# smdogroup/eigd

Measured on AMD Instinct MI355X. Metric: adjoint_mode_derivatives_per_sec, higher is better.
Workload: dtype f64

## Files before the change

### eigd_amd/csrc/sparse.hip

```cpp
#include <algorithm>
#include <cstdint>
#include <vector>

#include "common.h"

struct eigd_mat {
  eigd_ctx* ctx = nullptr;
  int n = 0;
  int ncols = 0;
  int64_t nnz = 0;
  int32_t* indptr = nullptr;
  int32_t* indices = nullptr;
  double* data = nullptr;
  int32_t* rowblocks = nullptr;
  int nblocks = 0;
  int ntiles = 0, umax = 0;
  int tnz_cap = 0;
  int32_t* tile_ptr = nullptr;
  int32_t* ucols = nullptr;
  uint16_t* lidx = nullptr;
};

namespace eigd {

constexpr int kTileRows = 32;
constexpr int kTileLds = 40 * 1024;
constexpr int kTileNnz = 1024;
constexpr int kNnzTile = 2048;
constexpr int kMaxRowsTile = 256;


__device__ __forceinline__ int xcd_remap(int b, int nblocks_padded) {
  const int per = nblocks_padded >> 3;
  return (b & 7) * per + (b >> 3);
}

__global__ __launch_bounds__(kThreads) void spmv_stream_kernel(const int32_t* __restrict__ rowblocks, int nblocks,
                                                              int nblocks_padded,
                                                              const int32_t* __restrict__ indptr,
                                                              const int32_t* __restrict__ indices,
                                                              const double* __restrict__ vals,
                                                              const double* __restrict__ x, double* __restrict__ y,
                                                              double alpha, double beta) {
  __shared__ double prod[kNnzTile];
  __shared__ double red[kThreads];
  const int b = xcd_remap(blockIdx.x, nblocks_padded);
  if (b >= nblocks) return;
  const int tid = threadIdx.x;
  const int r0 = rowblocks[b], r1 = rowblocks[b + 1];
  const int e0 = indptr[r0], e1 = indptr[r1];
  if (e1 - e0 <= kNnzTile - 2) {
    constexpr int IT = kNnzTile / (2 * kThreads);
    const int eb = e0 & ~1;
    typedef double dbl2 __attribute__((ext_vector_type(2)));
    typedef int int2v __attribute__((ext_vector_type(2)));
    dbl2 v[IT];
    int2v col[IT];
    double xa[IT], xb[IT];
#pragma unroll
    for (int it = 0; it < IT; ++it) {
      const int e = eb + 2 * (tid + it * kThreads);
      if (e < e1) {
        v[it] = __builtin_nontemporal_load(reinterpret_cast<const dbl2*>(vals + e));
        col[it] = __builtin_nontemporal_load(reinterpret_cast<const int2v*>(indices + e));
      } else {
        v[it] = dbl2{0.0, 0.0};
        col[it] = int2v{0, 0};
      }
    }
#pragma unroll
    for (int it = 0; it < IT; ++it) {
      const int e = eb + 2 * (tid + it * kThreads);
      xa[it] = (e >= e0 && e < e1) ? x[col[it][0]] : 0.0;
      xb[it] = (e + 1 < e1) ? x[col[it][1]] : 0.0;
    }
#pragma unroll
    for (int it = 0; it < IT; ++it) {
      const int e = eb + 2 * (tid + it * kThreads);
      if (e >= e0 && e < e1) prod[e - e0] = __dmul_rn(v[it][0], xa[it]);
      if (e + 1 < e1) prod[e + 1 - e0] = __dmul_rn(v[it][1], xb[it]);
    }
    __syncthreads();
    for (int r = r0 + tid; r < r1; r += kThreads) {
      const int a = indptr[r] - e0, z = indptr[r + 1] - e0;
      double s = 0.0;
      for (int q = a; q < z; ++q) s = __dadd_rn(s, prod[q]);
      y[r] = (beta == 0.0) ? alpha * s : alpha * s + beta * y[r];
    }
  } else {
    double s = 0.0;
    for (int e = e0 + tid; e < e1; e += kThreads) s += vals[e] * x[indices[e]];
    red[tid] = s;
    __syncthreads();
    for (int w = kThreads / 2; w > 0; w >>= 1) {
      if (tid < w) red[tid] += red[tid + w];
      __syncthreads();
    }
    if (tid == 0) y[r0] = (beta == 0.0) ? alpha * red[0] : alpha * red[0] + beta * y[r0];
  }
}

template <int KP>
__global__ __launch_bounds__(kThreads) void spmm_rows_kernel(int n, int k, const int32_t* __restrict__ indptr,
                                                            const int32_t* __restrict__ indices,
                                                            const double* __restrict__ vals,
                                                            const double* __restrict__ X, int ldx,
                                                            double* __restrict__ Y, int ldy, double alpha,
                                                            double beta) {
  constexpr int RP = kThreads / KP;
  const int c = threadIdx.x % KP;
  const int r = blockIdx.x * RP + threadIdx.x / KP;
  if (r >= n || c >= k) return;
  const int a = indptr[r], z = indptr[r + 1];
  double s = 0.0;
  int e = a;
  for (; e + 8 <= z; e += 8) {
    int col[8];
    double v[8], x[8];
#pragma unroll
    for (int q = 0; q < 8; ++q) {
      col[q] = indices[e + q];
      v[q] = vals[e + q];
    }
#pragma unroll
    for (int q = 0; q < 8; ++q) x[q] = X[static_cast<int64_t>(col[q]) * ldx + c];
#pragma unroll
    for (int q = 0; q < 8; ++q) s = __dadd_rn(s, __dmul_rn(v[q], x[q]));
  }
  for (; e < z; ++e) s = __dadd_rn(s, __dmul_rn(vals[e], X[static_cast<int64_t>(indices[e]) * ldx + c]));
  double* yp = Y + static_cast<int64_t>(r) * ldy + c;
  *yp = (beta == 0.0) ? alpha * s : alpha * s + beta * (*yp);
}

template <int KP, int LANES = 8>
struct SpmmTile {
  static constexpr int CPL = (KP >= LANES) ? KP / LANES : 1;
  static constexpr int LPR = KP / CPL;
  static constexpr int LD = (CPL >= 2) ? KP + 4 : KP + 1;
};

template <int KP, int LANES, bool DOTS = false>
__global__ __launch_bounds__(kThreads) void spmm_tiled_kernel(int n, int k, int ntiles, int tiles_per_xcd,
                                                             const int32_t* __restrict__ tile_ptr,
                                                             const int32_t* __restrict__ ucols,
                                                             const int32_t* __restrict__ indptr,
                                                             const uint16_t* __restrict__ lidx,
                                                             const double* __restrict__ vals,
                                                             const double* __restrict__ X, int ldx,
                                                             double* __restrict__ Y, int ldy, double alpha, double beta,
                                                             int umax, int tnz_cap,
                                                             const double* __restrict__ R = nullptr, int ldr = 0,
                                                             double* __restrict__ dots = nullptr) {
  extern __shared__ __align__(16) double Xs[];
  constexpr int RP = kThreads / KP;
  constexpr int CPL = SpmmTile<KP, LANES>::CPL, LPR = SpmmTile<KP, LANES>::LPR, LD = SpmmTile<KP, LANES>::LD;
  constexpr int RPP = kThreads / LPR;
  constexpr int NR = (kTileRows + RPP - 1) / RPP;
  double* const Vs = Xs + static_cast<size_t>(umax) * LD;
  uint16_t* const Ls = reinterpret_cast<uint16_t*>(Vs + tnz_cap);
  const int tile = (blockIdx.x & 7) * tiles_per_xcd + (blockIdx.x >> 3);
  if (tile >= ntiles) return;
  const int c = threadIdx.x % KP, rr = threadIdx.x / KP;
  const int pl = threadIdx.x % LPR, prow = threadIdx.x / LPR;
  const int u0 = tile_ptr[tile], nu = tile_ptr[tile + 1] - u0;
  const int rend = min(n, (tile + 1) * kTileRows);
  const int e0 = indptr[tile * kTileRows], tnz = indptr[rend] - e0;
  const bool staged = tnz <= tnz_cap;
  constexpr int NQ = kTileNnz / kThreads;
  int ra[NR], rz[NR];
#pragma unroll
  for (int i = 0; i < NR; ++i) {
    const int r = tile * kTileRows + prow + i * RPP;
    ra[i] = (r < rend) ? indptr[r] - e0 : 0;
    rz[i] = (r < rend) ? indptr[r + 1] - e0 : 0;
  }
  double sv[NQ];
  uint16_t sl[NQ];
#pragma unroll
  for (int q = 0; q < NQ; ++q) {
    const int e = threadIdx.x + q * kThreads;
    const bool ok = staged && e < tnz;
    sv[q] = ok ? vals[e0 + e] : 0.0;
    sl[q] = ok ? lidx[e0 + e] : uint16_t(0);
  }
  [[maybe_unused]] double xo[CPL], ro[CPL];
  if constexpr (DOTS) {
    const int r = tile * kTileRows + prow;
#pragma unroll
    for (int t = 0; t < CPL; ++t) {
      const bool ok = r < rend && CPL * pl + t < k;
      xo[t] = ok ? X[static_cast<int64_t>(r) * ldx + CPL * pl + t] : 0.0;
      ro[t] = ok ? R[static_cast<int64_t>(r) * ldr + CPL * pl + t] : 0.0;
    }
  }
  constexpr int SU = 16;
  for (int j0 = 0; j0 < nu; j0 += SU * RP) {
    int col[SU];
    double x[SU];
#pragma unroll
    for (int q = 0; q < SU; ++q) {
      const int j = j0 + q * RP + rr;
      col[q] = (j < nu) ? ucols[u0 + j] : -1;
    }
#pragma unroll
    for (int q = 0; q < SU; ++q) x[q] = (col[q] >= 0 && c < k) ? X[static_cast<int64_t>(col[q]) * ldx + c] : 0.0;
#pragma unroll
    for (int q = 0; q < SU; ++q) {
      const int j = j0 + q * RP + rr;
      if (j < nu) Xs[j * LD + c] = x[q];
    }
  }
  if (staged) {
#pragma unroll
    for (int q = 0; q < NQ; ++q) {
      const int e = threadIdx.x + q * kThreads;
      if (e < tnz) {
        Vs[e] = sv[q];
        Ls[e] = sl[q];
      }
    }
  }
  __syncthreads();
  const int cb = CPL * pl;
  if (!DOTS && cb >= k) return;
  [[maybe_unused]] double dzr[CPL], dzy[CPL];
  [[maybe_unused]] __shared__ double dred[DOTS ? (kThreads / 64) * 2 * KP : 1];
  if constexpr (DOTS) {
#pragma unroll
    for (int t = 0; t < CPL; ++t) dzr[t] = dzy[t] = 0.0;
  }
  auto finish_dots = [&]() {
    if constexpr (DOTS) {
      static_assert(KP >= LANES && NR == 1, "one pass over the tile's rows, eight lanes per row");
#pragma unroll
      for (int t = 0; t < CPL; ++t) {
#pragma unroll
        for (int off = LPR; off < 64; off <<= 1) {
          dzr[t] += __shfl_xor(dzr[t], off, 64);
          dzy[t] += __shfl_xor(dzy[t], off, 64);
        }
      }
      const int wave = threadIdx.x >> 6, lane = threadIdx.x & 63;
      if (lane < LPR) {
#pragma unroll
        for (int t = 0; t < CPL; ++t) {
          dred[(wave * 2 + 0) * KP + cb + t] = dzr[t];
          dred[(wave * 2 + 1) * KP + cb + t] = dzy[t];
        }
      }
      __syncthreads();
      if (threadIdx.x < 2 * k) {
        const int q = threadIdx.x / k, c2 = threadIdx.x % k;
        double v = 0.0;
#pragma unroll
        for (int w = 0; w < kThreads / 64; ++w) v += dred[(w * 2 + q) * KP + c2];
        dots[static_cast<int64_t>(tile) * 2 * k + threadIdx.x] = v;
      }
    }
  };
  auto store_row = [&](int r, const double (&s)[CPL]) {
    double* yp = Y + static_cast<int64_t>(r) * ldy + cb;
#pragma unroll
    for (int t = 0; t < CPL; ++t)
      if (cb + t < k) {
        const double yv = (beta == 0.0) ? alpha * s[t] : alpha * s[t] + beta * yp[t];
        yp[t] = yv;
        if constexpr (DOTS) {
          dzr[t] += xo[t] * ro[t];
          dzy[t] += xo[t] * yv;
        }
      }
  };
  const bool active = cb < k;
  if (active && staged) {
#pragma unroll
    for (int i = 0; i < NR; ++i) {
      const int r = tile * kTileRows + prow + i * RPP;
      if (r >= rend) break;
      const int a = ra[i], z = rz[i];
      double s[CPL];
#pragma unroll
      for (int t = 0; t < CPL; ++t) s[t] = 0.0;
      int e = a;
      for (; e + 8 <= z; e += 8) {
        int li[8];
        double v[8], x[8][CPL];
#pragma unroll
        for (int q = 0; q < 8; ++q) {
          li[q] = Ls[e + q];
          v[q] = Vs[e + q];
        }
#pragma unroll
        for (int q = 0; q < 8; ++q) {
          const double* xp = Xs + li[q] * LD + cb;
          if constexpr (CPL >= 2) {
            const double2* xp2 = reinterpret_cast<const double2*>(xp);
#pragma unroll
            for (int t = 0; t < CPL / 2; ++t) {
              const double2 w = xp2[t];
              x[q][2 * t] = w.x;
              x[q][2 * t + 1] = w.y;
            }
          } else {
            x[q][0] = xp[0];
          }
        }
#pragma unroll
        for (int q = 0; q < 8; ++q)
#pragma unroll
          for (int t = 0; t < CPL; ++t) s[t] = __dadd_rn(s[t], __dmul_rn(v[q], x[q][t]));
      }
      for (; e < z; ++e) {
        const double v = Vs[e];
        const double* xp = Xs + Ls[e] * LD + cb;
#pragma unroll
        for (int t = 0; t < CPL; ++t) s[t] = __dadd_rn(s[t], __dmul_rn(v, xp[t]));
      }
      store_row(r, s);
    }
  } else if (active) {
  for (int r = tile * kTileRows + prow; r < rend; r += RPP) {
    const int a = indptr[r], z = indptr[r + 1];
    double s[CPL];
#pragma unroll
    for (int t = 0; t < CPL; ++t) s[t] = 0.0;
    for (int e = a; e < z; ++e) {
      const double v = vals[e];
      const double* xp = Xs + lidx[e] * LD + cb;
#pragma unroll
      for (int t = 0; t < CPL; ++t) s[t] = __dadd_rn(s[t], __dmul_rn(v, xp[t]));
    }
    store_row(r, s);
  }
  }
  finish_dots();
}

__global__ __launch_bounds__(kThreads) void tile_dots_reduce_kernel(const double* __restrict__ dots, int ntiles, int nout,
                                                                   double* __restrict__ out) {
  __shared__ double red[kThreads];
  const int per = kThreads / nout;
  const int o = threadIdx.x % nout, sub = threadIdx.x / nout;
  double v = 0.0;
  if (sub < per)
    for (int t = blockIdx.x * per + sub; t < ntiles; t += gridDim.x * per) v += dots[static_cast<int64_t>(t) * nout + o];
  red[threadIdx.x] = v;
  __syncthreads();
  if (threadIdx.x < nout) {
    double t = 0.0;
    for (int q = 0; q < per; ++q) t += red[q * nout + threadIdx.x];
    out[static_cast<int64_t>(blockIdx.x) * nout + threadIdx.x] = t;
  }
}

}

using namespace eigd;

extern "C" {

int eigd_csr_upload(eigd_ctx* ctx, int n, int64_t nnz, const int32_t* hindptr, const int32_t* hindices,
                    const double* hdata, eigd_mat** out) {
  return eigd_csr_upload_rect(ctx, n, n, nnz, hindptr, hindices, hdata, out);
}

int eigd_csr_upload_rect(eigd_ctx* ctx, int n, int ncols, int64_t nnz, const int32_t* hindptr, const int32_t* hindices,
                         const double* hdata, eigd_mat** out) {
  EIGD_REQUIRE(ctx && hindptr && hindices && hdata && out, "null argument");
  EIGD_REQUIRE(n > 0 && ncols > 0 && nnz >= 0 && nnz < (int64_t(1) << 31), "bad matrix size %d x %d nnz=%lld", n, ncols,
               (long long)nnz);
  EIGD_REQUIRE(hindptr[0] == 0 && hindptr[n] == nnz, "indptr does not match nnz");
  for (int i = 0; i < n; ++i) EIGD_REQUIRE(hindptr[i + 1] >= hindptr[i], "indptr not monotone at row %d", i);
  for (int64_t e = 0; e < nnz; ++e)
    EIGD_REQUIRE(hindices[e] >= 0 && hindices[e] < ncols, "column index out of range at entry %lld", (long long)e);
  *out = nullptr;
  std::vector<int32_t> rb;
  rb.push_back(0);
  {
    int r = 0;
    while (r < n) {
      int start = r;
      int64_t cnt = 0;
      while (r < n && (r - start) < kMaxRowsTile) {
        int64_t len = hindptr[r + 1] - hindptr[r];
        if (cnt + len > kNnzTile - 2) break;
        cnt += len;
        ++r;
      }
      if (r == start) ++r;
      rb.push_back(r);
    }
  }
  const int ntiles = (n + kTileRows - 1) / kTileRows;
  std::vector<int32_t> tile_ptr(static_cast<size_t>(ntiles) + 1, 0), ucols;
  std::vector<uint16_t> lidx(static_cast<size_t>(nnz) + 8, 0);
  int umax = 0;
  int64_t tnz_max = 0;
  bool tiles_ok = true;
  {
    std::vector<int32_t> cols, stamp(static_cast<size_t>(ncols), -1), pos(static_cast<size_t>(ncols), 0);
    ucols.reserve(static_cast<size_t>(nnz) / 4 + 16);
    for (int t = 0; t < ntiles && tiles_ok; ++t) {
      const int r0 = t * kTileRows, r1 = std::min(n, r0 + kTileRows);
      cols.clear();
      for (int64_t e = hindptr[r0]; e < hindptr[r1]; ++e) {
        const int32_t cidx = hindices[e];
        if (stamp[cidx] != t) {
          stamp[cidx] = t;
          cols.push_back(cidx);
        }
      }
      std::sort(cols.begin(), cols.end());
      if (cols.size() > 65535) tiles_ok = false;
      umax = std::max<int>(umax, static_cast<int>(cols.size()));
      tnz_max = std::max<int64_t>(tnz_max, hindptr[r1] - hindptr[r0]);
      for (size_t q = 0; q < cols.size(); ++q) pos[cols[q]] = static_cast<int32_t>(q);
      for (int64_t e = hindptr[r0]; e < hindptr[r1]; ++e) lidx[e] = static_cast<uint16_t>(pos[hindices[e]]);
      ucols.insert(ucols.end(), cols.begin(), cols.end());
      tile_ptr[t + 1] = static_cast<int32_t>(ucols.size());
    }
  }
  EIGD_HIP(hipSetDevice(ctx->device));
  eigd_mat* A = new eigd_mat();
  A->ctx = ctx;
  A->n = n;
  A->ncols = ncols;
  A->nnz = nnz;
  A->nblocks = static_cast<int>(rb.size()) - 1;
  if (tiles_ok) {
    A->ntiles = ntiles;
    A->umax = umax;
    A->tnz_cap = static_cast<int>(std::min<int64_t>(kTileNnz, (tnz_max + 7) & ~int64_t(7)));
    hipError_t t1 = hipMalloc(reinterpret_cast<void**>(&A->tile_ptr), sizeof(int32_t) * tile_ptr.size());
    hipError_t t2 = hipMalloc(reinterpret_cast<void**>(&A->ucols), sizeof(int32_t) * std::max<size_t>(ucols.size(), 1));
    hipError_t t3 = hipMalloc(reinterpret_cast<void**>(&A->lidx), sizeof(uint16_t) * lidx.size());
    if (t1 != hipSuccess || t2 != hipSuccess || t3 != hipSuccess) {
      eigd_mat_free(A);
      set_error("hipMalloc failed for the SpMM tiles (n=%d nnz=%lld)", n, (long long)nnz);
      return EIGD_E_HIP;
    }
    EIGD_HIP(hipMemcpy(A->tile_ptr, tile_ptr.data(), sizeof(int32_t) * tile_ptr.size(), hipMemcpyHostToDevice));
    if (!ucols.empty()) EIGD_HIP(hipMemcpy(A->ucols, ucols.data(), sizeof(int32_t) * ucols.size(), hipMemcpyHostToDevice));
    EIGD_HIP(hipMemcpy(A->lidx, lidx.data(), sizeof(uint16_t) * lidx.size(), hipMemcpyHostToDevice));
  }
  hipError_t e1 = hipMalloc(reinterpret_cast<void**>(&A->indptr), sizeof(int32_t) * (n + 1));
  hipError_t e2 = hipMalloc(reinterpret_cast<void**>(&A->indices), sizeof(int32_t) * (nnz + 4));
  hipError_t e3 = hipMalloc(reinterpret_cast<void**>(&A->data), sizeof(double) * (nnz + 4));
  hipError_t e4 = hipMalloc(reinterpret_cast<void**>(&A->rowblocks), sizeof(int32_t) * rb.size());
  if (e1 != hipSuccess || e2 != hipSuccess || e3 != hipSuccess || e4 != hipSuccess) {
    eigd_mat_free(A);
    set_error("hipMalloc failed for CSR matrix (n=%d nnz=%lld)", n, (long long)nnz);
    return EIGD_E_HIP;
  }
  EIGD_HIP(hipMemcpy(A->indptr, hindptr, sizeof(int32_t) * (n + 1), hipMemcpyHostToDevice));
  if (nnz > 0) {
    EIGD_HIP(hipMemcpy(A->indices, hindices, sizeof(int32_t) * nnz, hipMemcpyHostToDevice));
    EIGD_HIP(hipMemcpy(A->data, hdata, sizeof(double) * nnz, hipMemcpyHostToDevice));
  }
  EIGD_HIP(hipMemcpy(A->rowblocks, rb.data(), sizeof(int32_t) * rb.size(), hipMemcpyHostToDevice));
  *out = A;
  return EIGD_OK;
}

int eigd_csr_update_values(eigd_mat* A, const double* hdata) {
  EIGD_REQUIRE(A && hdata, "null argument");
  EIGD_HIP(hipStreamSynchronize(A->ctx->stream));
  if (A->nnz > 0) EIGD_HIP(hipMemcpy(A->data, hdata, sizeof(double) * A->nnz, hipMemcpyHostToDevice));
  return EIGD_OK;
}

int eigd_csr_update_values_dev(eigd_mat* A, const double* dvals) {
  EIGD_REQUIRE(A && dvals, "null argument");
  if (A->nnz > 0)
    EIGD_HIP(hipMemcpyAsync(A->data, dvals, sizeof(double) * A->nnz, hipMemcpyDeviceToDevice, A->ctx->stream));
  return EIGD_OK;
}

int eigd_mat_free(eigd_mat* A) {
  if (!A) return EIGD_OK;
  if (A->ctx && A->ctx->stream) (void)hipStreamSynchronize(A->ctx->stream);
  if (A->indptr) (void)hipFree(A->indptr);
  if (A->indices) (void)hipFree(A->indices);
  if (A->data) (void)hipFree(A->data);
  if (A->rowblocks) (void)hipFree(A->rowblocks);
  if (A->tile_ptr) (void)hipFree(A->tile_ptr);
  if (A->ucols) (void)hipFree(A->ucols);
  if (A->lidx) (void)hipFree(A->lidx);
  delete A;
  return EIGD_OK;
}

int eigd_spmm(eigd_mat* A, const double* dX, int ldx, double* dY, int ldy, int k, double alpha, double beta) {
  EIGD_REQUIRE(A, "null argument");
  return eigd_spmm_on(A->ctx, A, dX, ldx, dY, ldy, k, alpha, beta);
}

int eigd_spmm_on(eigd_ctx* ctx, eigd_mat* A, const double* dX, int ldx, double* dY, int ldy, int k, double alpha,
                 double beta) {
  EIGD_REQUIRE(ctx && A && dX && dY, "null argument");
  EIGD_REQUIRE(ctx->device == A->ctx->device, "context and matrix live on different devices");
  EIGD_REQUIRE(k >= 1 && ldx >= k && ldy >= k, "bad block shape k=%d ldx=%d ldy=%d", k, ldx, ldy);
  EIGD_REQUIRE(dX != dY, "spmm cannot run in place");
  hipStream_t st = ctx->stream;
  if (k == 1 && ldx == 1 && ldy == 1) {
    const int nbp = (A->nblocks + 7) & ~7;
    hipLaunchKernelGGL(spmv_stream_kernel, dim3(nbp), dim3(kThreads), 0, st, A->rowblocks, A->nblocks, nbp, A->indptr,
                       A->indices, A->data, dX, dY, alpha, beta);
    EIGD_LAUNCH_CHECK();
    return EIGD_OK;
  }
  auto tile_fits = [&](int kpv) {
    const int cplv = (kpv >= 8) ? kpv / 8 : 1;
    return A->ntiles > 0 && sizeof(double) * static_cast<size_t>(A->umax) * (cplv >= 2 ? kpv + 4 : kpv + 1) <= static_cast<size_t>(kTileLds);
  };
  const int chunk = (k > 32 && !tile_fits(64) && tile_fits(32)) ? 32 : kMaxK;
  for (int c0 = 0; c0 < k; c0 += chunk) {
    const int kb = std::min(chunk, k - c0);
    const int kp = std::max(2, next_pow2(kb));
    const int rp = kThreads / kp;
    const dim3 grid((A->n + rp - 1) / rp);
    const int cpl = (kp >= 8) ? kp / 8 : 1;
    const size_t tile_lds = sizeof(double) * static_cast<size_t>(A->umax) * (cpl >= 2 ? kp + 4 : kp + 1);
    const size_t tile_lds_all = tile_lds + static_cast<size_t>(A->tnz_cap) * (sizeof(double) + sizeof(uint16_t));
    if (A->ntiles > 0 && tile_lds <= static_cast<size_t>(kTileLds)) {
      const int per_xcd = (A->ntiles + 7) / 8;
      const dim3 tgrid(per_xcd * 8);
#define EIGD_SPMM_TILED(KP)                                                                                            \
  case KP:                                                                                                             \
    hipLaunchKernelGGL((spmm_tiled_kernel<KP, 8>), tgrid, dim3(kThreads), tile_lds_all, st, A->n, kb, A->ntiles,       \
                       per_xcd, A->tile_ptr, A->ucols, A->indptr, A->lidx, A->data, dX + c0, ldx, dY + c0, ldy,        \
                       alpha, beta, A->umax, A->tnz_cap);                                                              \
    break;
      switch (kp) {
        EIGD_SPMM_TILED(2)
        EIGD_SPMM_TILED(4)
        EIGD_SPMM_TILED(8)
        EIGD_SPMM_TILED(16)
        EIGD_SPMM_TILED(32)
        EIGD_SPMM_TILED(64)
        default:
          set_error("internal: unexpected kp=%d", kp);
          return EIGD_E_INTERNAL;
      }
#undef EIGD_SPMM_TILED
      EIGD_LAUNCH_CHECK();
      continue;
    }
#define EIGD_SPMM_CASE(KP)                                                                                          \
  case KP:                                                                                                          \
    hipLaunchKernelGGL(spmm_rows_kernel<KP>, grid, dim3(kThreads), 0, st, A->n, kb, A->indptr, A->indices, A->data, \
                       dX + c0, ldx, dY + c0, ldy, alpha, beta);                                                    \
    break;
    switch (kp) {
      EIGD_SPMM_CASE(2)
      EIGD_SPMM_CASE(4)
      EIGD_SPMM_CASE(8)
      EIGD_SPMM_CASE(16)
      EIGD_SPMM_CASE(32)
      EIGD_SPMM_CASE(64)
      default:
        set_error("internal: unexpected kp=%d", kp);
        return EIGD_E_INTERNAL;
    }
#undef EIGD_SPMM_CASE
    EIGD_LAUNCH_CHECK();
  }
  return EIGD_OK;
}

int eigd_spmm_cg(eigd_ctx* ctx, eigd_mat* A, int k, const double* dZ, int ldz, double* dY, int ldy, const double* dR, int ldr,
                 const double* dNorm2, double* dState, int step, int first, double* dLog) {
  EIGD_REQUIRE(ctx && A && dZ && dY && dR && dState, "null argument");
  EIGD_REQUIRE(ctx->device == A->ctx->device, "context and matrix live on different devices");
  EIGD_REQUIRE(k >= 1 && k <= kMaxK && ldz >= k && ldy >= k && ldr >= k && A->n == A->ncols, "bad block shape k=%d", k);
  EIGD_REQUIRE(dZ != dY, "spmm cannot run in place");
  const int kp = std::max(2, next_pow2(k));
  const int cpl = (kp >= 8) ? kp / 8 : 1;
  const size_t tile_lds = sizeof(double) * static_cast<size_t>(A->umax) * (cpl >= 2 ? kp + 4 : kp + 1);
  const bool fused = kp >= 8 && kp <= 32 && A->ntiles > 0 && tile_lds <= static_cast<size_t>(kTileLds);
  if (!fused) {
    int rc = eigd_spmm_on(ctx, A, dZ, ldz, dY, ldy, k, 1.0, 0.0);
    if (rc) return rc;
    return eigd_cg_coefficients(ctx, A->n, k, dZ, ldz, dR, ldr, dY, ldy, dNorm2, dState, step, first, dLog);
  }
  const int groups = std::min(A->ntiles, 1024);
  int rc = ctx->ensure_scratch(sizeof(double) * (static_cast<size_t>(A->ntiles) + groups) * 2 * k);
  if (rc) return rc;
  double* gsum = ctx->scratch;
  double* dots = ctx->scratch + static_cast<size_t>(groups) * 2 * k;
  const size_t tile_lds_all = tile_lds + static_cast<size_t>(A->tnz_cap) * (sizeof(double) + sizeof(uint16_t));
  const int per_xcd = (A->ntiles + 7) / 8;
  const dim3 tgrid(per_xcd * 8);
  hipStream_t st = ctx->stream;
#define EIGD_SPMM_DOTS(KP)                                                                                             \
  case KP:                                                                                                             \
    hipLaunchKernelGGL((spmm_tiled_kernel<KP, 8, true>), tgrid, dim3(kThreads), tile_lds_all, st, A->n, k, A->ntiles,  \
                       per_xcd, A->tile_ptr, A->ucols, A->indptr, A->lidx, A->data, dZ, ldz, dY, ldy, 1.0, 0.0,        \
                       A->umax, A->tnz_cap, dR, ldr, dots);                                                            \
    break;
  switch (kp) {
    EIGD_SPMM_DOTS(8)
    EIGD_SPMM_DOTS(16)
    EIGD_SPMM_DOTS(32)
    default:
      set_error("internal: unexpected kp=%d", kp);
      return EIGD_E_INTERNAL;
  }
#undef EIGD_SPMM_DOTS
  EIGD_LAUNCH_CHECK();
  hipLaunchKernelGGL(tile_dots_reduce_kernel, dim3(groups), dim3(kThreads), 0, st, dots, A->ntiles, 2 * k, gsum);
  EIGD_LAUNCH_CHECK();
  return cg_coefficients_from_partials(ctx, gsum, groups, k, dNorm2, dState, step, first, dLog);
}

}
```

Measured before the change: 667.5.

## Pad per-tile column lists and hoist gather loads ahead of value staging

Replaces the tile_ptr indirection with a fixed-stride padded ucols array, so each tile's column list starts at tile*umax and the dependent tile_ptr load disappears. The first batch of column indices and X gathers is issued before the vals/lidx staging loads, and those loads are made unconditional through clamped indices so more memory requests are in flight at once. The gather batch size now adapts to rows per pass. In exchange, padded tiles gather up to umax columns even when the tile holds fewer, which adds wasted work on irregular matrices. A host check also disables tiling when padding would inflate memory too much.

```diff
diff --git a/eigd_amd/csrc/sparse.hip b/eigd_amd/csrc/sparse.hip
--- a/eigd_amd/csrc/sparse.hip
+++ b/eigd_amd/csrc/sparse.hip
@@ -16,7 +16,6 @@
   int nblocks = 0;
   int ntiles = 0, umax = 0;
   int tnz_cap = 0;
-  int32_t* tile_ptr = nullptr;
   int32_t* ucols = nullptr;
   uint16_t* lidx = nullptr;
 };
@@ -141,7 +140,6 @@
 
 template <int KP, int LANES, bool DOTS = false>
 __global__ __launch_bounds__(kThreads) void spmm_tiled_kernel(int n, int k, int ntiles, int tiles_per_xcd,
-                                                             const int32_t* __restrict__ tile_ptr,
                                                              const int32_t* __restrict__ ucols,
                                                              const int32_t* __restrict__ indptr,
                                                              const uint16_t* __restrict__ lidx,
@@ -162,53 +160,69 @@
   if (tile >= ntiles) return;
   const int c = threadIdx.x % KP, rr = threadIdx.x / KP;
   const int pl = threadIdx.x % LPR, prow = threadIdx.x / LPR;
-  const int u0 = tile_ptr[tile], nu = tile_ptr[tile + 1] - u0;
-  const int rend = min(n, (tile + 1) * kTileRows);
-  const int e0 = indptr[tile * kTileRows], tnz = indptr[rend] - e0;
-  const bool staged = tnz <= tnz_cap;
+  const int32_t* const tcols = ucols + static_cast<int64_t>(tile) * umax;
+  const int rbeg = tile * kTileRows, rend = min(n, rbeg + kTileRows);
+  const int e0 = indptr[rbeg], tnz = indptr[rend] - e0;
   constexpr int NQ = kTileNnz / kThreads;
   int ra[NR], rz[NR];
 #pragma unroll
   for (int i = 0; i < NR; ++i) {
-    const int r = tile * kTileRows + prow + i * RPP;
-    ra[i] = (r < rend) ? indptr[r] - e0 : 0;
-    rz[i] = (r < rend) ? indptr[r + 1] - e0 : 0;
-  }
+    const int r = rbeg + prow + i * RPP;
+    ra[i] = indptr[min(r, rend)];
+    rz[i] = indptr[min(r + 1, rend)];
+  }
+  constexpr int SU = (256 / RP < 1) ? 1 : (256 / RP > 16) ? 16 : 256 / RP;
+  int col[SU];
+  auto load_cols = [&](int j0) {
+#pragma unroll
+    for (int q = 0; q < SU; ++q) {
+      const int j = j0 + q * RP + rr;
+      const int v = tcols[max(0, min(j, umax - 1))];
+      col[q] = (j < umax) ? v : -1;
+    }
+  };
+  load_cols(0);
+  [[maybe_unused]] double xo[CPL], ro[CPL];
+  if constexpr (DOTS) {
+    const int r = rbeg + prow;
+#pragma unroll
+    for (int t = 0; t < CPL; ++t) {
+      const bool ok = r < rend && CPL * pl + t < k;
+      const int64_t rc = min(r, rend - 1), cc = min(CPL * pl + t, k - 1);
+      const double xv = X[rc * ldx + cc], rv = R[rc * ldr + cc];
+      xo[t] = ok ? xv : 0.0;
+      ro[t] = ok ? rv : 0.0;
+    }
+  }
+  double x[SU];
+  auto load_x = [&]() {
+#pragma unroll
+    for (int q = 0; q < SU; ++q) x[q] = (col[q] >= 0 && c < k) ? X[static_cast<int64_t>(col[q]) * ldx + c] : 0.0;
+  };
+  auto store_x = [&](int j0) {
+#pragma unroll
+    for (int q = 0; q < SU; ++q)
+      if (col[q] >= 0) Xs[(j0 + q * RP + rr) * LD + c] = x[q];
+  };
+  load_x();
+  const bool staged = tnz <= tnz_cap;
   double sv[NQ];
   uint16_t sl[NQ];
 #pragma unroll
   for (int q = 0; q < NQ; ++q) {
     const int e = threadIdx.x + q * kThreads;
     const bool ok = staged && e < tnz;
-    sv[q] = ok ? vals[e0 + e] : 0.0;
-    sl[q] = ok ? lidx[e0 + e] : uint16_t(0);
-  }
-  [[maybe_unused]] double xo[CPL], ro[CPL];
-  if constexpr (DOTS) {
-    const int r = tile * kTileRows + prow;
-#pragma unroll
-    for (int t = 0; t < CPL; ++t) {
-      const bool ok = r < rend && CPL * pl + t < k;
-      xo[t] = ok ? X[static_cast<int64_t>(r) * ldx + CPL * pl + t] : 0.0;
-      ro[t] = ok ? R[static_cast<int64_t>(r) * ldr + CPL * pl + t] : 0.0;
-    }
-  }
-  constexpr int SU = 16;
-  for (int j0 = 0; j0 < nu; j0 += SU * RP) {
-    int col[SU];
-    double x[SU];
-#pragma unroll
-    for (int q = 0; q < SU; ++q) {
-      const int j = j0 + q * RP + rr;
-      col[q] = (j < nu) ? ucols[u0 + j] : -1;
-    }
-#pragma unroll
-    for (int q = 0; q < SU; ++q) x[q] = (col[q] >= 0 && c < k) ? X[static_cast<int64_t>(col[q]) * ldx + c] : 0.0;
-#pragma unroll
-    for (int q = 0; q < SU; ++q) {
-      const int j = j0 + q * RP + rr;
-      if (j < nu) Xs[j * LD + c] = x[q];
-    }
+    const int ec = e0 + max(0, min(e, tnz - 1));
+    const double v = vals[ec];
+    const uint16_t l = lidx[ec];
+    sv[q] = ok ? v : 0.0;
+    sl[q] = ok ? l : uint16_t(0);
+  }
+  store_x(0);
+  for (int j0 = SU * RP; j0 < umax; j0 += SU * RP) {
+    load_cols(j0);
+    load_x();
+    store_x(j0);
   }
   if (staged) {
 #pragma unroll
@@ -275,9 +289,9 @@
   if (active && staged) {
 #pragma unroll
     for (int i = 0; i < NR; ++i) {
-      const int r = tile * kTileRows + prow + i * RPP;
+      const int r = rbeg + prow + i * RPP;
       if (r >= rend) break;
-      const int a = ra[i], z = rz[i];
+      const int a = ra[i] - e0, z = rz[i] - e0;
       double s[CPL];
 #pragma unroll
       for (int t = 0; t < CPL; ++t) s[t] = 0.0;
@@ -420,6 +434,10 @@
       tile_ptr[t + 1] = static_cast<int32_t>(ucols.size());
     }
   }
+  const int64_t ucols_padded = static_cast<int64_t>(ntiles) * umax;
+  if (sizeof(double) * 3 * static_cast<int64_t>(umax) > kTileLds ||
+      ucols_padded > std::max<int64_t>(2 * static_cast<int64_t>(ucols.size()), (16 << 20) / sizeof(int32_t)))
+    tiles_ok = false;
   EIGD_HIP(hipSetDevice(ctx->device));
   eigd_mat* A = new eigd_mat();
   A->ctx = ctx;
@@ -431,16 +449,17 @@
     A->ntiles = ntiles;
     A->umax = umax;
     A->tnz_cap = static_cast<int>(std::min<int64_t>(kTileNnz, (tnz_max + 7) & ~int64_t(7)));
-    hipError_t t1 = hipMalloc(reinterpret_cast<void**>(&A->tile_ptr), sizeof(int32_t) * tile_ptr.size());
-    hipError_t t2 = hipMalloc(reinterpret_cast<void**>(&A->ucols), sizeof(int32_t) * std::max<size_t>(ucols.size(), 1));
-    hipError_t t3 = hipMalloc(reinterpret_cast<void**>(&A->lidx), sizeof(uint16_t) * lidx.size());
-    if (t1 != hipSuccess || t2 != hipSuccess || t3 != hipSuccess) {
+    std::vector<int32_t> padded(static_cast<size_t>(std::max<int64_t>(ucols_padded, 1)), -1);
+    for (int t = 0; t < ntiles; ++t)
+      std::copy(ucols.begin() + tile_ptr[t], ucols.begin() + tile_ptr[t + 1], padded.begin() + static_cast<size_t>(t) * umax);
+    hipError_t t1 = hipMalloc(reinterpret_cast<void**>(&A->ucols), sizeof(int32_t) * padded.size());
+    hipError_t t2 = hipMalloc(reinterpret_cast<void**>(&A->lidx), sizeof(uint16_t) * lidx.size());
+    if (t1 != hipSuccess || t2 != hipSuccess) {
       eigd_mat_free(A);
       set_error("hipMalloc failed for the SpMM tiles (n=%d nnz=%lld)", n, (long long)nnz);
       return EIGD_E_HIP;
     }
-    EIGD_HIP(hipMemcpy(A->tile_ptr, tile_ptr.data(), sizeof(int32_t) * tile_ptr.size(), hipMemcpyHostToDevice));
-    if (!ucols.empty()) EIGD_HIP(hipMemcpy(A->ucols, ucols.data(), sizeof(int32_t) * ucols.size(), hipMemcpyHostToDevice));
+    EIGD_HIP(hipMemcpy(A->ucols, padded.data(), sizeof(int32_t) * padded.size(), hipMemcpyHostToDevice));
     EIGD_HIP(hipMemcpy(A->lidx, lidx.data(), sizeof(uint16_t) * lidx.size(), hipMemcpyHostToDevice));
   }
   hipError_t e1 = hipMalloc(reinterpret_cast<void**>(&A->indptr), sizeof(int32_t) * (n + 1));
@@ -483,7 +502,6 @@
   if (A->indices) (void)hipFree(A->indices);
   if (A->data) (void)hipFree(A->data);
   if (A->rowblocks) (void)hipFree(A->rowblocks);
-  if (A->tile_ptr) (void)hipFree(A->tile_ptr);
   if (A->ucols) (void)hipFree(A->ucols);
   if (A->lidx) (void)hipFree(A->lidx);
   delete A;
@@ -528,7 +546,7 @@
 #define EIGD_SPMM_TILED(KP)                                                                                            \
   case KP:                                                                                                             \
     hipLaunchKernelGGL((spmm_tiled_kernel<KP, 8>), tgrid, dim3(kThreads), tile_lds_all, st, A->n, kb, A->ntiles,       \
-                       per_xcd, A->tile_ptr, A->ucols, A->indptr, A->lidx, A->data, dX + c0, ldx, dY + c0, ldy,        \
+                       per_xcd, A->ucols, A->indptr, A->lidx, A->data, dX + c0, ldx, dY + c0, ldy,        \
                        alpha, beta, A->umax, A->tnz_cap);                                                              \
     break;
       switch (kp) {
@@ -595,7 +613,7 @@
 #define EIGD_SPMM_DOTS(KP)                                                                                             \
   case KP:                                                                                                             \
     hipLaunchKernelGGL((spmm_tiled_kernel<KP, 8, true>), tgrid, dim3(kThreads), tile_lds_all, st, A->n, k, A->ntiles,  \
-                       per_xcd, A->tile_ptr, A->ucols, A->indptr, A->lidx, A->data, dZ, ldz, dY, ldy, 1.0, 0.0,        \
+                       per_xcd, A->ucols, A->indptr, A->lidx, A->data, dZ, ldz, dY, ldy, 1.0, 0.0,        \
                        A->umax, A->tnz_cap, dR, ldr, dots);                                                            \
     break;
   switch (kp) {
```

New measurement: 671.9, median of 6. No clear change (+0.7%).
